# Nextomics/NextPolish2

Hardware: AMD Instinct MI355X
Metric: polished reference Mbp/s (whole node) at 30x HiFi + k21/k31; FASTA identical to oracle (higher is better)
Workload: dtype u8

## Files before the change

### nextpolish2_amd/csrc/np2_ctx.hpp

```cpp
#pragma once
#include "../../include/np2.h"
#include "np2_abi.hpp"
#include "np2_common.hpp"
#include "np2_kernels.hpp"
#include "np2_hostcpu.hpp"

#include <algorithm>
#include <chrono>
#include <cstdio>
#include <cstdlib>
#include <cstring>
#include <map>
#include <memory>
#include <exception>
#include <mutex>
#include <stdexcept>
#include <string>
#include <vector>

namespace np2h {

using namespace np2;


// ... 446 lines not shown
    DevBuf<uint16_t> keep_ks;
    DevBuf<uint32_t> long_list;
    DevBuf<uint64_t> bt_path;
    DevBuf<uint64_t> chunk_st;
    uint32_t chunk_epoch = 0;
    DevBuf<uint32_t> tile_cur, tile_n, tile_scan, tile_scanb, tile_nn, tile_nr, tile_noff, tile_roff;
    uint32_t tile_cap = TILE_CAP;
    uint32_t bucket_cap = 0;
    DevBuf<uint2> nrec;
    DevBuf<uint8_t> votebuf;
    DevBuf<uint32_t> band, band_n, band_off, row_cnt;
    DevBuf<int64_t> run_gain, tile_gain;
    DevBuf<uint8_t> out_snap;
    DevBuf<uint8_t> run_flag;
    uint32_t deep_min = 65536;
    DevBuf<uint32_t> lq_list, hbits;
    DevBuf<uint16_t> tile_pidx;
    bool pidx_valid = false;
    DevBuf<ReadInfo> rinfo;
    DevBuf<uint32_t> lqc, lqoff;
    DevBuf<uint8_t> pflag;
    DevBuf<uint32_t> dp_list;
    DevBuf<uint16_t> pf_slots;
    DevBuf<uint32_t> pf_bad, pf_bad2;
    DevBuf<uint64_t> pf_prof;
    bool front_fused = false;
    struct Hooks {
        bool front_unfused = false, pf_prof = false, edge_sort = false;
        bool test_misspeculate = false, shard_spec_log = false, phase_profile = false, exact_grow = false, no_speculate = false;
        bool has_grow_guess = false;
        uint32_t grow_guess = 0;
        bool has_pf_cap = false, has_pf_cap_big = false, has_pf_halo = false, has_pf_cov_max = false;
        uint32_t pf_cap = 0, pf_cap_big = 0, pf_halo = 0, pf_cov_max = 0;
        void read() {
            auto on = [](const char *n) { return getenv(n) != nullptr; };
            auto u32 = [](const char *n, bool &has, uint32_t &v) {
                if (const char *e = getenv(n)) has = true, v = (uint32_t)atol(e);
            };
            front_unfused = on("NP2_FRONT_UNFUSED"), pf_prof = on("NP2_PF_PROF"), edge_sort = on("NP2_EDGE_SORT");
            test_misspeculate = on("NP2_TEST_MISSPECULATE");
            shard_spec_log = on("NP2_SHARD_SPEC_LOG"), phase_profile = on("NP2_PHASE_PROFILE"), exact_grow = on("NP2_EXACT_GROW");
            no_speculate = on("NP2_NO_SPECULATE");
            u32("NP2_TEST_GROW_GUESS", has_grow_guess, grow_guess);
            u32("NP2_PF_CAP", has_pf_cap, pf_cap), u32("NP2_PF_CAP_BIG", has_pf_cap_big, pf_cap_big);
            u32("NP2_PF_HALO", has_pf_halo, pf_halo), u32("NP2_PF_COV_MAX", has_pf_cov_max, pf_cov_max);
        }
    } hooks;
    bool pf_big = getenv("NP2_PF_BIG") != nullptr;
    uint32_t front_redos = 0;
    DevBuf<uint16_t> kscore_saved;
    DevBuf<uint8_t> sstr;
    DevBuf<uint64_t> soff;
    DevBuf<uint16_t> sscore;
};


namespace np2h {


enum Scal { S_ERR = 0, S_NNODES, S_NRUNS, S_BEST, S_PATHBEGIN, S_NRAW, S_NREG, S_DUP, S_LAST0, S_LAST1, S_GAIN0,
            S_GAIN1, S_DEEP, S_NDPLIST, S_NRECH, S_NGROUPS, S_NLONG, S_NLQ, S_PF, S_M0, S_M1, S_M2, S_M3, S_NC, S_SB, S_GROW,
            S_NBAD, S_PFOUT, S_PFGAIN0, S_PFGAIN1, S_PFEND0, S_PFEND1, S_NBAD2, S_NOKEY, S_COUNT = 34 };
static_assert(S_M1 % 2 == 0 && S_LAST0 % 2 == 0 && S_GAIN0 % 2 == 0 && S_PFGAIN0 % 2 == 0 && S_PFEND0 % 2 == 0,
              "64-bit device counters live in these slot pairs");

static constexpr int NP2_MAX_YAK = 15;
static constexpr uint32_t SCAL_TOTAL = 96;
static_assert(S_COUNT + 2 * (NP2_MAX_YAK + 2) <= SCAL_TOTAL && S_COUNT < 64, "round counters behind the posted block; the mailbox holds 64 words");

inline double thread_cpu_ms() {
    timespec ts;
    clock_gettime(CLOCK_THREAD_CPUTIME_ID, &ts);
    return ts.tv_sec * 1e3 + ts.tv_nsec * 1e-6;
}
struct WallTimer {
    np2_ctx *cx;
    const char *name;
    double t0, c0 = 0;
    WallTimer(np2_ctx *c, const char *n);
    ~WallTimer();
};

struct EventTimer {
    np2_ctx *cx;
    hipEvent_t a = nullptr, b = nullptr;
    bool on;
    EventTimer(np2_ctx *c, const char *name, bool always = false)
        : cx(c), on((always || c->stage_timing) && !tl_recorder()) {
        if (!on) return;
        (void)hipEventCreate(&a);
        (void)hipEventCreate(&b);
        (void)hipEventRecord(a, cx->stream);
        cx->pending_events.push_back({name, {a, b}});
    }
    ~EventTimer() {
// ... 233 lines not shown
```

### nextpolish2_amd/csrc/np2_graph.hip

```cpp
#include "np2_common.hpp"
#include "np2_kernels.hpp"
#include "np2_blockscan.hpp"
#include "np2_lookback.hpp"

namespace np2 {

__device__ __forceinline__ uint32_t block_excl_scan_256(uint32_t v, uint32_t *sh, uint32_t &total) {
    return block_excl_scan<OpAdd, 4>(v, sh, total);
}

__device__ uint64_t make_node_key(const np2_read_t *__restrict__ reads, const uint8_t *__restrict__ nib, uint64_t rec,
                                  uint32_t r) {
    const uint32_t col = (uint32_t)rec, t3 = (uint32_t)(rec >> 32);
    const np2_read_t rd = reads[r];
    const uint8_t *base = nib + rd.nib_off;
    const uint32_t ts = rd.aln_t_s;
    auto mk = [&](int64_t c, uint32_t t) -> AlignBase {
        if (c == -2) return ab_head(ts - 1, 0);
        if (c == -1) return ab_head(ts - 1, 1);
        const uint8_t nb = nib_at(base, (uint32_t)c);
        AlignBase a;
        a.q = nb & 7;
        a.t_pos = t;
        a.delta = 0;
        if (c > 0 && (nb & 8)) {
            uint16_t dl = 1;
            int64_t x = c - 1;
            while (x > 0 && (nib_at(base, (uint32_t)x) & 8)) {
                dl = (uint16_t)(dl + 1);
                --x;
            }
            a.delta = dl;
        }
        return a;
    };
    auto is_ins = [&](int64_t c) -> bool { return c > 0 && (nib_at(base, (uint32_t)c) & 8); };
    const int64_t c3 = col;
    const AlignBase b3 = mk(c3, t3);
    const uint32_t t2 = is_ins(c3) ? t3 : t3 - 1;
    const AlignBase b2 = mk(c3 - 1, t2);
    const uint32_t t1 = is_ins(c3 - 1) ? t2 : t2 - 1;
    const AlignBase b1 = mk(c3 - 2, t1);
    return ((uint64_t)b3.t_pos << 32) | ((uint64_t)node_bases(b1, b2, b3) << 16) | b1.delta;
}

__device__ __forceinline__ void k_tile_layout(const uint32_t np2_bid, const uint32_t np2_nb, uint32_t *__restrict__ tile_cur, uint32_t n_tiles,
                                                      uint32_t bucket_cap, uint32_t *__restrict__ tile_n,
                                                      uint32_t *__restrict__ tile_scan, uint32_t *__restrict__ tile_scanb,
                                                      const uint32_t *__restrict__ ovf_cnt, uint32_t *__restrict__ out) {
    __shared__ uint32_t sh[16];
    const uint32_t ta = block_scan_array<OpAdd>(
        n_tiles, sh, [&](uint32_t i) { return tile_cur[i]; },
        [&](uint32_t i, uint32_t pre, uint32_t v) {
            tile_scan[i] = pre;
            tile_n[i] = v;
        });
    const uint32_t tb = block_scan_array<OpAdd>(
        n_tiles, sh, [&](uint32_t i) { return min(tile_n[i], bucket_cap); },
        [&](uint32_t i, uint32_t pre, uint32_t) { tile_scanb[i] = pre; });
    const uint32_t mx = block_scan_array<OpMaxU32>(
        n_tiles, sh, [&](uint32_t i) { return tile_n[i]; }, [&](uint32_t i, uint32_t, uint32_t) { tile_cur[i] = 0; });
    if (threadIdx.x == 0) {
        tile_scan[n_tiles] = ta;
        tile_scanb[n_tiles] = tb;
        out[0] = ta;
        out[1] = mx;
        out[2] = *ovf_cnt;
    }
}

static constexpr uint32_t TLB_ITEMS = 4;
__device__ __forceinline__ void k_tile_layout_lb(const uint32_t np2_bid, const uint32_t np2_nb, Lookback lb, uint32_t n_blocks, uint32_t *__restrict__ tile_cur,
                                                        uint32_t n_tiles, uint32_t bucket_cap, uint32_t *__restrict__ tile_n,
                                                        uint32_t *__restrict__ tile_scan, uint32_t *__restrict__ tile_scanb,
                                                        const uint32_t *__restrict__ ovf_cnt, uint32_t *__restrict__ out,
                                                        uint32_t *__restrict__ err) {
// ... 67 lines not shown
        s_klo[i] = (uint32_t)k;
        s_v[i] = r;
        s_q[i] = (uint16_t)q;
        atomicAdd(&s_cnt[q], 1u);
    }
    __syncthreads();
    {
        const uint32_t q0 = tid * 4;
        const uint32_t c0 = s_cnt[q0], c1 = s_cnt[q0 + 1], c2 = s_cnt[q0 + 2], c3 = s_cnt[q0 + 3];
        uint32_t tot;
        const uint32_t l0 = block_excl_scan_256(c0 + c1 + c2 + c3, sh, tot);
        s_off[q0] = (uint16_t)l0, s_off[q0 + 1] = (uint16_t)(l0 + c0), s_off[q0 + 2] = (uint16_t)(l0 + c0 + c1), s_off[q0 + 3] = (uint16_t)(l0 + c0 + c1 + c2);
        s_cnt[q0] = 0, s_cnt[q0 + 1] = 0, s_cnt[q0 + 2] = 0, s_cnt[q0 + 3] = 0;
    }
    __syncthreads();
    for (uint32_t i = tid; i < n; i += 256) {
        const uint32_t q = s_q[i];
        s_idx[s_off[q] + atomicAdd(&s_cnt[q], 1u)] = (uint16_t)i;
    }
    if (tid < TILE / 16) pidx[(size_t)np2_bid * (TILE / 16) + tid] = s_off[tid * 16];
    __syncthreads();
    for (uint32_t d = tid; d < n; d += 256) {
        const uint32_t i = s_idx[d], q = s_q[i], b = s_off[q], m = s_cnt[q];
        const uint32_t klo = s_klo[i], v = s_v[i];
        uint32_t rank = 0;
        for (uint32_t e = b; e < b + m; ++e) {
            const uint32_t j = s_idx[e];
            const uint32_t kj = s_klo[j], vj = s_v[j];
            rank += (kj < klo || (kj == klo && vj < v)) ? 1u : 0u;
        }
        keys[a + b + rank] = ((uint64_t)(start + q) << 32) | klo;
        vals[a + b + rank] = v;
    }
}

__device__ __forceinline__ void k_gather_buckets(const uint32_t np2_bid, const uint32_t np2_nb, const np2_read_t *__restrict__ reads,
                                                        const uint8_t *__restrict__ nib,
                                                        const uint32_t *__restrict__ tile_n,
                                                        const uint32_t *__restrict__ tile_scanb, uint32_t bucket_cap,
                                                        const uint64_t *__restrict__ bkeys,
                                                        const uint32_t *__restrict__ bvals, uint64_t *__restrict__ keys,
                                                        uint32_t *__restrict__ vals) {
    const uint32_t n = min(tile_n[np2_bid], bucket_cap);
    const uint64_t a = (uint64_t)np2_bid * bucket_cap;
    const uint32_t dst = tile_scanb[np2_bid];
    for (uint32_t i = threadIdx.x; i < n; i += 256) {
        const uint32_t r = bvals[a + i];
        keys[dst + i] = make_node_key(reads, nib, bkeys[a + i], r);
        vals[dst + i] = r;
    }
}
__device__ __forceinline__ void k_gather_spill(const uint32_t np2_bid, const uint32_t np2_nb, const np2_read_t *__restrict__ reads, const uint8_t *__restrict__ nib,
                               const uint64_t *__restrict__ okeys, const uint32_t *__restrict__ ovals, uint32_t n,
                               uint64_t *__restrict__ keys, uint32_t *__restrict__ vals) {
    const uint32_t i = np2_bid * blockDim.x + threadIdx.x;
    if (i >= n) return;
    const uint32_t r = ovals[i];
    keys[i] = make_node_key(reads, nib, okeys[i], r);
    vals[i] = r;
}

__device__ __forceinline__ bool group_head(const uint64_t *__restrict__ keys, const uint32_t *__restrict__ vals,
                                           const uint8_t *__restrict__ alive, uint64_t i, uint64_t a, uint64_t b,
                                           uint32_t &cnt, uint32_t &mn) {
    const uint64_t k = keys[i];
    if (i > a && keys[i - 1] == k) return false;
// ... 456 lines not shown
                if (q0 + j < npos) {
                    cov[start + q0 + j] = cv[j];
                    node_off[start + q0 + j] = nbase + off[j];
                    emit[start + q0 + j] = em[j];
                }
        }
    }
    if (np2_bid == n_tiles - 1 && tid == 255) node_off[L] = nbase + off[4];
    if (max(max(cv[0], cv[1]), max(cv[2], cv[3])) >= deep_min) atomicOr(deep_flag, 1u);
    if (tid == 0) tile_gain[np2_bid] = s_gain[0] + s_gain[1] + s_gain[2] + s_gain[3];
    if (fast) {
        for (uint32_t i = tid; i < nn; i += 256) {
            const uint32_t kk = s_nkey[i], c = s_ncnt[i];
            const uint32_t o = nbase + i;
            nd.bases[o] = (uint16_t)(kk >> 16);
            nd.delta[o] = (uint16_t)kk;
            nd.count[o] = c;
            nrec[o] = make_uint2((kk >> 16) | (kk << 16), c);
        }
    }
}

uint32_t tile_scan_blocks(uint32_t n_tiles) { return (n_tiles + 256 * TLB_ITEMS - 1) / (256 * TLB_ITEMS); }
void launch_tile_layout(hipStream_t s, uint32_t *tile_cur, uint32_t n_tiles, uint32_t bucket_cap, uint32_t *tile_n,
                        uint32_t *tile_scan, uint32_t *tile_scanb, const uint32_t *ovf_cnt, uint32_t *out,
                        const Lookback *lb, uint32_t *err) {
    if (lb)
        NP2_LAUNCH(k_tile_layout_lb, dim3(tile_scan_blocks(n_tiles)), 256, s, *lb, tile_scan_blocks(n_tiles), tile_cur, n_tiles, bucket_cap, tile_n, tile_scan, tile_scanb, ovf_cnt, out, err);
    else
        NP2_LAUNCH(k_tile_layout, dim3(1), 1024, s, tile_cur, n_tiles, bucket_cap, tile_n, tile_scan, tile_scanb, ovf_cnt, out);
}
void launch_tile_sort(hipStream_t s, uint16_t *pidx, const np2_read_t *reads, const uint8_t *nib, const uint32_t *tile_n,
                      uint32_t n_tiles, uint32_t bucket_cap, uint32_t max_tile, uint64_t *keys, uint32_t *vals,
                      uint32_t *err) {
    const uint32_t ALL = 0xFFFFFFFFu;
    if (max_tile <= 1024) {
        NP2_LAUNCH(k_tile_sort<1024>, dim3(n_tiles), 256, s, pidx, reads, nib, tile_n, bucket_cap, keys, vals, err, 0u, ALL);
    } else {
        NP2_LAUNCH(k_tile_sort<1024>, dim3(n_tiles), 256, s, pidx, reads, nib, tile_n, bucket_cap, keys, vals, err, 0u, 1024u);
        if (max_tile <= 2048 && TILE_CAP > 2048)
            NP2_LAUNCH(k_tile_sort<2048>, dim3(n_tiles), 256, s, pidx, reads, nib, tile_n, bucket_cap, keys, vals, err, 1024u, ALL);
        else
            NP2_LAUNCH(k_tile_sort<TILE_CAP>, dim3(n_tiles), 256, s, pidx, reads, nib, tile_n, bucket_cap, keys, vals, err, 1024u, ALL);
    }
}
void launch_gather_buckets(hipStream_t s, const np2_read_t *reads, const uint8_t *nib, const uint32_t *tile_n,
                           const uint32_t *tile_scanb, uint32_t n_tiles, uint32_t bucket_cap, const uint64_t *bkeys,
                           const uint32_t *bvals, uint64_t *keys, uint32_t *vals) {
    NP2_LAUNCH(k_gather_buckets, dim3(n_tiles), 256, s, reads, nib, tile_n, tile_scanb, bucket_cap, bkeys, bvals, keys, vals);
}
void launch_gather_spill(hipStream_t s, const np2_read_t *reads, const uint8_t *nib, const uint64_t *okeys,
                         const uint32_t *ovals, uint32_t n, uint64_t *keys, uint32_t *vals) {
    if (n) NP2_LAUNCH(k_gather_spill, dim3((n + 255) / 256), 256, s, reads, nib, okeys, ovals, n, keys, vals);
}
void launch_tile_count(hipStream_t s, const uint64_t *keys, const uint32_t *vals, const uint32_t *tile_n,
                       const uint32_t *tile_scan, uint32_t bucket_cap, uint32_t n_tiles, const uint8_t *alive,
                       uint32_t *tile_nn, uint32_t *tile_nr) {
    NP2_LAUNCH(k_tile_count, dim3(n_tiles), 256, s, keys, vals, TileLayout{tile_n, tile_scan, bucket_cap}, alive, tile_nn, tile_nr);
}
void launch_tile_offsets(hipStream_t s, const uint32_t *tile_nn, const uint32_t *tile_nr, uint32_t n_tiles,
                         uint32_t *tile_noff, uint32_t *tile_roff, uint32_t *n_nodes, uint32_t *n_runs, uint32_t *reset,
                         uint32_t n_reset, const Lookback *lb, uint32_t *err, const long long *tile_gain,
                         unsigned long long *gain_total) {
    if (lb)
        NP2_LAUNCH(k_tile_offsets_lb, dim3(tile_scan_blocks(n_tiles)), 256, s, *lb, tile_scan_blocks(n_tiles), tile_nn, tile_nr, n_tiles, tile_noff, tile_roff, n_nodes, n_runs, reset, n_reset, err, tile_gain, gain_total);
    else
        NP2_LAUNCH(k_tile_offsets, dim3(1), 1024, s, tile_nn, tile_nr, n_tiles, tile_noff, tile_roff, n_nodes, n_runs, reset, n_reset, tile_gain, gain_total);
}
void launch_tile_write(hipStream_t s, const uint64_t *keys, const uint32_t *vals, const uint32_t *tile_n,
                       const uint32_t *tile_scan, uint32_t bucket_cap, const uint32_t *tile_noff, const uint32_t *tile_roff,
                       uint32_t n_tiles, const uint8_t *alive, uint32_t L, NodeArrays nd, uint2 *nrec, uint32_t *node_off,
                       uint32_t *run_start, const np2_read_t *reads, const uint32_t *tile_rd_off, const uint32_t *tile_rd,
                       int32_t *cov, const uint8_t *refnib, uint32_t *emit, long long *tile_gain, uint32_t *deep_flag, uint32_t deep_min,
                       uint8_t *pflag) {
    NP2_LAUNCH(k_tile_write, dim3(n_tiles), 256, s, keys, vals, TileLayout{tile_n, tile_scan, bucket_cap}, tile_noff, tile_roff, alive, L, n_tiles, nd, nrec, node_off, run_start, reads, tile_rd_off, tile_rd, cov, refnib, emit, tile_gain, deep_flag, (int32_t)deep_min, pflag);
}
// ... 3 lines not shown
```

### nextpolish2_amd/csrc/np2_host.cpp

```cpp
#include "../../include/np2.h"
#include "np2_common.hpp"
#include "np2_kernels.hpp"
#include "np2_ctx.hpp"
#include "np2_phase_host.hpp"

#include <algorithm>
#include <atomic>
#include <thread>
#include <chrono>
#include <cstdio>
#include <cstdlib>
#include <cstring>
#include <map>
#include <mutex>
#include <stdexcept>
#include <string>
#include <unordered_map>
#include <unordered_set>
#include <future>
#include <functional>
#include <vector>

using namespace np2;

// ... 617 lines not shown
            launch_diff_reads(s, c->descs.p, NCH, c->nib.p, (const uint64_t *)c->refnib.p, c->refnib.p, c->refnib.p + c->ref_stride, c->ref_stride, L,
                              cx->keys_raw.p, cx->vals_raw.p, cx->tile_cur.p, n_tiles, bcap, buckets, (uint32_t)ovf_cap,
                              cx->scal.p + S_M3, c->ckpt.p, cx->chunk_st.p, cx->chunk_epoch, cx->scal.p + S_ERR);
        }
        {
            EventTimer t(cx, "sort_exceptions");
            const bool wide = n_tiles >= 2048;
            Lookback lb{};
            if (wide) lb = next_lookback(cx, tile_scan_blocks(n_tiles));
            launch_tile_layout(s, cx->tile_cur.p, n_tiles, bcap, cx->tile_n.p, cx->tile_scan.p, cx->tile_scanb.p,
                               cx->scal.p + S_M3, cx->scal.p + S_M0, wide ? &lb : nullptr, cx->scal.p + S_ERR);
        }
        std::vector<uint32_t> sc = fetch_scal(cx);
        static const bool test_fail = getenv("NP2_TEST_DENSE_LB_FAIL") != nullptr;
        if (test_fail && attempt == 0 && !precount) sc[S_ERR] |= LB_ERR;
        if ((sc[S_ERR] & LB_ERR) && !precount) {
            precount = true;
            continue;
        }
        if (sc[S_ERR] & ~2u) check_region_err(cx, sc[S_ERR] & ~2u);
        if (sc[S_ERR] & 2u)
            throw Np2Error(NP2_E_ARG, "packed read inconsistent with its descriptor (n_cols / aln_t_e / terminator)");
        if (sc[S_M2] > ovf_cap) {
            ovf_cap = (uint64_t)sc[S_M2] * 5 / 4 + 65536;
            continue;
        }
        T = sc[S_M0];
        if (T >= 0xFFFFFFF0u) throw Np2Error(NP2_E_NOMEM, "too many exception nodes");
        cx->tmp.ensure(prim_temp_bytes(std::max<size_t>({(size_t)T + 1, (size_t)L + 2, (size_t)R + 1})));
        EventTimer t(cx, "sort_exceptions");
        if (sc[S_M2] == 0) {
            cx->tile_pidx.ensure((size_t)n_tiles * (TILE / 16) + 64);
            launch_tile_sort(s, cx->tile_pidx.p, c->reads.p, c->nib.p, cx->tile_n.p, n_tiles, bcap, sc[S_M1], cx->keys_raw.p,
                             cx->vals_raw.p, cx->scal.p + S_ERR);
            cx->bucket_cap = bcap;
            cx->pidx_valid = true;
        } else {
            cx->keys.ensure((size_t)T + 1);
            cx->vals.ensure((size_t)T + 1);
            const uint32_t nb = T - sc[S_M2];
            launch_gather_buckets(s, c->reads.p, c->nib.p, cx->tile_n.p, cx->tile_scanb.p, n_tiles, bcap, cx->keys_raw.p,
                                  cx->vals_raw.p, cx->keys.p, cx->vals.p);
            launch_gather_spill(s, c->reads.p, c->nib.p, cx->keys_raw.p + buckets, cx->vals_raw.p + buckets, sc[S_M2],
                                cx->keys.p + nb, cx->vals.p + nb);
            unsigned pos_bits = 1;
            while ((1ull << pos_bits) < (uint64_t)L + 1) ++pos_bits;
            prim_op(cx, [=](hipStream_t st) {
                if (prim_sort_pairs_u64_u32(st, cx->tmp.p, cx->tmp.cap, cx->keys.p, cx->keys_raw.p, cx->vals.p, cx->vals_raw.p,
                                            T, 32 + pos_bits))
                    throw Np2Error(NP2_E_DEVICE, "rocprim radix_sort_pairs failed");
            });
            cx->bucket_cap = 0;
            cx->pidx_valid = false;
        }
        return;
    }
    throw Np2Error(NP2_E_NOMEM, "exception buffer kept overflowing");
}

void build_graph(np2_ctx *cx, np2_contig *c, uint32_t T, uint32_t &n_nodes, uint32_t &n_runs) {
    hipStream_t s = cx->stream;
    const uint32_t L = c->L;
    const uint32_t n_tiles = (L + TILE - 1) >> TILE_SHIFT;
    EventTimer t(cx, "build_graph");
    cx->npos.ensure(T + 1);
    cx->nbases.ensure(T + 1);
    cx->ndelta.ensure(T + 1);
// ... 192 lines not shown
        launch_pf_tile(s, a);
        if (prof) {
            auto st = d2h(cx, cx->pf_prof.p, (size_t)n_tiles * 8);
            double sum[8] = {0}, mx[8] = {0};
            size_t cnt = 0;
            for (uint32_t t = 0; t < n_tiles; ++t) {
                const uint64_t *q = st.data() + (size_t)t * 8;
                if (!q[7] || !q[0]) continue;
                ++cnt;
                for (int i = 1; i < 8; ++i) {
                    const double d = (double)(q[i] - q[i - 1]);
                    sum[i] += d, mx[i] = std::max(mx[i], d);
                }
            }
            {
                auto tn = d2h(cx, cx->tile_n.p, n_tiles);
                uint32_t h[6] = {0};
                for (uint32_t v : tn) ++h[v <= 480 ? 0 : v <= 960 ? 1 : v <= 1440 ? 2 : v <= 1920 ? 3 : v <= 3584 ? 4 : 5];
                fprintf(stderr, "[pf_prof] records per tile <=480 / 960 / 1440 / 1920 / 3584 / more: %u %u %u %u %u %u; ", h[0], h[1], h[2], h[3], h[4], h[5]);
            }
            fprintf(stderr, "listed for the middle / the big variant: %u / %u; ", d2h(cx, cx->scal.p + S_NBAD, 1)[0], d2h(cx, cx->scal.p + S_NBAD2, 1)[0]);
            fprintf(stderr, "tiles %zu of %u; mean / max clocks per phase (loads, cover+nodes, offsets+sort, DP, reduce, count+scan, write):", cnt, n_tiles);
            for (int i = 1; i < 8; ++i) fprintf(stderr, " %.0f/%.0f", cnt ? sum[i] / cnt : 0.0, mx[i]);
            fprintf(stderr, "\n");
        }
        const bool wide = n_tiles >= 2048;
        Lookback lb{};
        if (wide) lb = next_lookback(cx, tile_scan_blocks(n_tiles));
        launch_tile_offsets(s, cx->tile_nn.p, cx->tile_nr.p, n_tiles, cx->tile_noff.p, cx->tile_roff.p, M_p, n_lq,
                            cx->scal.p + S_BEST, S_NLQ + 1 - S_BEST, wide ? &lb : nullptr, cx->scal.p + S_ERR,
                            (const long long *)cx->tile_gain.p, (unsigned long long *)(cx->scal.p + S_PFGAIN0));
        launch_pf_compact(s, n_tiles, cx->pf_slots.p, cx->tile_scan.p, cx->tile_nn.p, cx->tile_noff.p, cx->tile_roff.p,
                          cx->cns_pos.p, cx->cns_base.p, cx->cns_cls.p, cx->lq_nothead.p, cx->lq_list.p, cb.lq_cap,
                          cx->scal.p + S_ERR, cx->scal.p + S_PF, cx->scal.p + S_PFOUT, cx->scal.p + S_NBAD, cx->scal.p + S_NBAD2);
    }
    lq_regions_issue(cx, cb, M_p, n_lq);
}

void pass_front_issue(np2_ctx *cx, np2_contig *c, uint32_t T, int pass, bool force_unfused = false) {
    cx->front_fused = !force_unfused && front_can_fuse(cx);
    if (!cx->front_fused || cx->trace) {
        uint32_t n_nodes = 0, n_runs = 0;
        {
            WallTimer w(cx, "wall_graph");
            build_graph(cx, c, T, n_nodes, n_runs);
        }
        trace_graph(cx, c, pass, n_nodes);
        if (!cx->front_fused) {
            consensus_and_regions_issue(cx, c, n_nodes, n_runs, T);
            return;
        }
    }
    pass_front_fused_issue(cx, c, T);
}
void consensus_and_regions_finish(np2_ctx *cx, np2_contig *c, uint32_t T, int pass, uint32_t &M, uint32_t &n_reg, bool whole_contig = true) {
    const uint32_t *M_p = cx->eoff.p + c->L;
    std::vector<uint32_t> sc = fetch_scal(cx, cx->scal.p + S_M0, M_p);
    if (cx->front_fused) {
        const int64_t total = (int64_t)(((uint64_t)sc[S_PFGAIN1] << 32) | sc[S_PFGAIN0]);
        const int64_t end_rel = (int64_t)(((uint64_t)sc[S_PFEND1] << 32) | sc[S_PFEND0]);
        const bool negative = end_rel <= SCORE_NEG / 2 || total + end_rel < 0;
        if (sc[S_PFOUT] & PF_NEED_BIG) cx->pf_big = true;
        if ((sc[S_PFOUT] & PF_REDO) || negative) {
            ++cx->front_redos;
            cx->timing.host.push_back({"front_redo", 1.0f});
            pass_front_issue(cx, c, T, pass, true);
            sc = fetch_scal(cx, cx->scal.p + S_M0, M_p);
        }
    }
    check_region_err(cx, sc[S_ERR]);
    if (!cx->front_fused && sc[S_BEST] == 0xFFFFFFFFu && !whole_contig)
        throw Np2Error(NP2_E_UNSUPPORTED,
                       "best path score is negative at the end of a shard (the reference's default node is chosen by the whole "
                       "contig's score): polish this contig unsharded");
    M = sc[S_M0];
    if (M == 0) throw Np2Error(NP2_E_REFPANIC, "reference would panic: empty consensus");
    n_reg = sc[S_NRAW] ? sc[S_NREG] : 0;
}

void extract_candidates(np2_ctx *cx, np2_contig *c, uint32_t n_reg, uint16_t min_kmer_count, int pass,
                        PassCounts &pc) {
    hipStream_t s = cx->stream;
    const uint32_t R = c->R;
    REFPANIC_IF(cx->yaks.empty(), "index out of bounds: opt.yak[0]");
    if ((uint64_t)n_reg * LQSEQ_MAX_CAN_COUNT >= 0xFFFFFFF0ull) throw Np2Error(NP2_E_NOMEM, "too many LQ regions");
    const uint32_t NC_cap = n_reg * LQSEQ_MAX_CAN_COUNT;
    static const uint64_t exact_from = getenv("NP2_CAND_EXACT_FROM") ? strtoull(getenv("NP2_CAND_EXACT_FROM"), nullptr, 10) : (1ull << 28);
    const bool exact_bytes = c->n_cols >= exact_from && !cx->trace;
    uint32_t SB_cap = (uint32_t)std::min<uint64_t>(c->n_cols + 64, 0xFFFFFFF0ull);
    cx->mval.ensure(R + 2);
    cx->smin.ensure(R + 2);
    cx->pj.ensure(R + 2);
    cx->pcount.ensure(R + 2);
    cx->rinfo.ensure(R + 2);
    cx->reg_ncand.ensure(n_reg + 2);
// ... 1372 lines not shown
```

### nextpolish2_amd/csrc/np2_kernels.hpp

```cpp
#pragma once
#include <cstddef>
#include <cstdint>
#include <hip/hip_runtime.h>
#include "../../include/np2.h"
#include "np2_lookback.hpp"
#include "np2_launch.hpp"

namespace np2 {

static constexpr uint32_t TILE_SHIFT = 10;
static constexpr uint32_t TILE = 1u << TILE_SHIFT;
static constexpr uint32_t TILE_CAP = 4096;

static constexpr uint32_t DENSE_COLS = 4096;
struct ChunkDesc {
    uint64_t nib_off;
    uint64_t ckbase;
    uint32_t read, ts;
    uint32_t c0, ncols;
    uint32_t first_chunk;
    uint32_t aln_t_e, nck;
    uint32_t pad0;
    uint32_t pad[4];
};
// ... 148 lines not shown
                          uint16_t min_count, uint16_t *out, bool own_strings);
void launch_cand_score(hipStream_t s, const YakDev &y, const uint32_t *cand_seq_off, const uint8_t *cand_seq,
                       const uint64_t *cand_kmer, const uint32_t *n_cand_p, uint32_t cand_cap, uint16_t min_count,
                       uint16_t *kscore, uint32_t *long_list, uint32_t *n_long);


void launch_pair_count(hipStream_t s, const np2_read_t *reads, uint32_t R, const uint8_t *alive,
                       const uint32_t *lq_start, const uint32_t *lq_end, uint32_t n_reg, const int32_t *smin,
                       uint32_t *pj, uint32_t *pcount, const uint64_t *ck_off, ReadInfo *rinfo);
void launch_scan_lb_excl(hipStream_t s, const Lookback &lb, const uint32_t *in, uint32_t *out, uint32_t n, bool write_end,
                          uint32_t *err);
uint32_t scan_lb_blocks(uint64_t n);
void launch_scan_small_excl(hipStream_t s, const uint32_t *in, uint32_t *out, uint32_t n, const uint32_t *n_dev,
                            uint32_t *total_out, bool write_end);
void launch_scan_small_incl(hipStream_t s, const int32_t *in, int32_t *out, uint32_t n, const uint32_t *n_dev);
void launch_scan_small_min(hipStream_t s, const int32_t *in, int32_t *out, uint32_t n, const uint32_t *n_dev);
void launch_region_measure(hipStream_t s, const CandPtrs &c, uint32_t n_reg, uint32_t *kept_read, uint32_t *kept_len,
                           uint32_t *kept_col, uint32_t *reg_ncand, uint32_t *reg_bytes, uint32_t *reg_maxlen,
                           uint32_t *blk_sum);
uint32_t cand_offsets_blocks(uint32_t n_reg);
void launch_cand_offsets(hipStream_t s, const uint32_t *blk_sum, uint32_t n_reg, uint32_t *blk_coff, uint32_t *blk_soff,
                         uint32_t *cand_off, uint32_t *reg_soff, uint32_t *n_cand, uint32_t *n_bytes, uint32_t *grow,
                         const Lookback *lb = nullptr, uint32_t *err = nullptr);
void launch_region_write(hipStream_t s, const CandPtrs &c, uint32_t n_reg, const uint32_t *kept_read,
                         const uint32_t *kept_len, const uint32_t *kept_col, const uint32_t *reg_ncand,
                         const uint32_t *reg_bytes, const uint32_t *blk_coff, const uint32_t *blk_soff, uint32_t *cand_off,
                         uint32_t *reg_soff, uint32_t cand_cap, uint32_t seq_cap, uint32_t *cand_order, uint64_t *cand_kmer,
                         uint32_t *cand_seq_off, uint8_t *cand_seq);

uint32_t tile_scan_blocks(uint32_t n_tiles);
void launch_tile_layout(hipStream_t s, uint32_t *tile_cur, uint32_t n_tiles, uint32_t bucket_cap, uint32_t *tile_n,
                        uint32_t *tile_scan, uint32_t *tile_scanb, const uint32_t *ovf_cnt, uint32_t *out,
                        const Lookback *lb = nullptr, uint32_t *err = nullptr);
void launch_tile_sort(hipStream_t s, uint16_t *pidx, const np2_read_t *reads, const uint8_t *nib, const uint32_t *tile_n,
                      uint32_t n_tiles, uint32_t bucket_cap, uint32_t max_tile, uint64_t *keys, uint32_t *vals,
                      uint32_t *err);
void launch_gather_buckets(hipStream_t s, const np2_read_t *reads, const uint8_t *nib, const uint32_t *tile_n,
                           const uint32_t *tile_scanb, uint32_t n_tiles, uint32_t bucket_cap, const uint64_t *bkeys,
                           const uint32_t *bvals, uint64_t *keys, uint32_t *vals);
void launch_gather_spill(hipStream_t s, const np2_read_t *reads, const uint8_t *nib, const uint64_t *okeys,
                         const uint32_t *ovals, uint32_t n, uint64_t *keys, uint32_t *vals);
void launch_tile_count(hipStream_t s, const uint64_t *keys, const uint32_t *vals, const uint32_t *tile_n,
                       const uint32_t *tile_scan, uint32_t bucket_cap, uint32_t n_tiles, const uint8_t *alive,
                       uint32_t *tile_nn, uint32_t *tile_nr);
void launch_tile_offsets(hipStream_t s, const uint32_t *tile_nn, const uint32_t *tile_nr, uint32_t n_tiles,
                         uint32_t *tile_noff, uint32_t *tile_roff, uint32_t *n_nodes, uint32_t *n_runs, uint32_t *reset,
                         uint32_t n_reset, const Lookback *lb = nullptr, uint32_t *err = nullptr,
                         const long long *tile_gain = nullptr, unsigned long long *gain_total = nullptr);
void launch_tile_write(hipStream_t s, const uint64_t *keys, const uint32_t *vals, const uint32_t *tile_n,
                       const uint32_t *tile_scan, uint32_t bucket_cap, const uint32_t *tile_noff, const uint32_t *tile_roff,
                       uint32_t n_tiles, const uint8_t *alive, uint32_t L, NodeArrays nd, uint2 *nrec, uint32_t *node_off,
                       uint32_t *run_start, const np2_read_t *reads, const uint32_t *tile_rd_off, const uint32_t *tile_rd,
                       int32_t *cov, const uint8_t *refnib, uint32_t *emit, long long *tile_gain, uint32_t *deep_flag, uint32_t deep_min,
                       uint8_t *pflag);

static constexpr uint32_t PF_CAP = 960;
static constexpr uint32_t PF_HALO = 64;
static constexpr uint32_t PF_CAP_MID = 2048;
static constexpr uint32_t PF_CAP_BIG = 3584;
static constexpr uint32_t PF_COV_MAX = 8192;
static constexpr uint32_t PF_REDO = 1u;
static constexpr uint32_t PF_NEED_BIG = 2u;
struct PfTile {
    const uint64_t *keys;
    const uint32_t *vals;
    const uint32_t *tile_n, *tile_scan;
    const uint16_t *pidx;
    const uint8_t *alive;
    const np2_read_t *reads;
    const uint32_t *tile_rd_off, *tile_rd;
    const uint8_t *refnib;
    uint16_t *slots;
    uint32_t *tile_cnt, *tile_lq;
    long long *tile_gain;
    uint32_t *flags, *n_bad, *bad_list, *n_bad2, *bad_list2;
    long long *end_rel;
    unsigned long long *gain_total;
    unsigned long long *prof;
    uint32_t L, n_tiles, bucket_cap;
    uint32_t cap_lim, cap_lim_big, halo_lim, cov_max;
    uint32_t big_enabled;
};
uint64_t pf_slot_entries(uint32_t n_tiles, uint64_t T);
void launch_pf_tile(hipStream_t s, const PfTile &a);
void launch_pf_compact(hipStream_t s, uint32_t n_tiles, const uint16_t *slots, const uint32_t *tile_scan, const uint32_t *tile_cnt,
                       const uint32_t *tile_coff, const uint32_t *tile_lqoff, uint32_t *cns_pos, uint8_t *cns_base,
                       uint8_t *cns_cls, uint8_t *lq_nothead, uint32_t *lq_list, uint32_t lq_cap, uint32_t *err, uint32_t *flags,
                       uint32_t *flags_out, uint32_t *n_bad, uint32_t *n_bad2);

struct RegionTables {
    const uint32_t *cand_off;
    const uint32_t *order;
    uint16_t *kscore;
    const uint32_t *seq_off;
    const uint8_t *seq;
    uint32_t n_reg;
};
struct RechPtrs {
    const void *groups;
    const uint32_t *job_off;
    const uint32_t *rech;
    const uint32_t *cand_off;
    const uint32_t *keep_list;
    const uint32_t *seq_off;
    const uint8_t *seq;
    const uint8_t *cns_base;
    uint32_t n_groups;
};
void launch_vote_phase(hipStream_t s, const RegionTables &rt, bool asref, bool use_all, const uint32_t *lq_start,
                       uint32_t own_lo, uint32_t own_hi, uint8_t *reg_lable, uint8_t *grp, uint32_t *ecount, int32_t *ref_w,
                       uint8_t *ref_seen, uint8_t *bad, uint32_t *first_reg, uint32_t *err);
void launch_vote_counts(hipStream_t s, const uint32_t *first_reg, const uint8_t *bad, uint32_t R, uint32_t *out);
void launch_edges_write(hipStream_t s, const RegionTables &rt, const uint8_t *reg_lable, const uint8_t *grp,
                        const uint32_t *ecount, const uint32_t *eoff, uint64_t *ekey, uint32_t *eval);
static constexpr uint32_t EDGE_BAND = 256;
void launch_edges_row(hipStream_t s, const RegionTables &rt, const uint8_t *grp, const uint32_t *ecount, const uint32_t *pj,
                      const uint32_t *pcount, const uint8_t *alive, uint32_t R, uint32_t *band, uint32_t *row_n, uint32_t *ovf);
void launch_band_emit(hipStream_t s, const uint32_t *band, uint32_t R, const uint32_t *row_off, uint64_t *ukey, uint32_t *uw,
                      uint32_t *n_out, uint64_t key_add = 0);
void launch_vote_rows_count(hipStream_t s, const uint32_t *band, const uint32_t *row_n, const uint8_t *bad, bool use_all, uint32_t R,
                            uint32_t *cnt, uint32_t *nokey);
// ... 66 lines not shown
```

### nextpolish2_amd/csrc/np2_passfront.hip

```cpp
#include "np2_common.hpp"
#include "np2_kernels.hpp"
#include "np2_blockscan.hpp"

namespace np2 {

static constexpr uint32_t PF_COUNT_BITS = 14;
static constexpr uint32_t PF_IDX_MASK = (1u << PF_COUNT_BITS) - 1;
static constexpr uint32_t PF_VISITED = 0x80000000u;
static constexpr uint32_t PF_N0_VISITED = 0x8000u;
static constexpr uint32_t PF_N0_WEAK = 0x4000u;
static constexpr uint32_t PF_N0_STRONG = 0x2000u;
static constexpr int32_t PF_NEG = -(1 << 30);

__device__ __forceinline__ uint8_t pf_ref_code(const uint8_t *__restrict__ refnib, uint32_t p) {
    return (refnib[p >> 1] >> (4 * (p & 1))) & 7;
}
template <int I> __device__ __forceinline__ uint32_t pf_quad_bcast(uint32_t v) {
    return (uint32_t)__builtin_amdgcn_mov_dpp((int)v, I | (I << 2) | (I << 4) | (I << 6), 0xF, 0xF, true);
}
__device__ __forceinline__ void pf_n0_key(uint32_t p, uint32_t c2, uint32_t c1, uint32_t c0, uint32_t &b, uint32_t &d) {
    if (p >= 2) {
        b = (c2 << 8) | (c1 << 4) | c0, d = 0;
    } else if (p == 1) {
        b = 0x0F00u | (c1 << 4) | c0, d = 1;
// ... 707 lines not shown
        A.tile_lq[t] = s_flag[3];
        A.tile_gain[t] = s_gain[0] + s_gain[1] + s_gain[2] + s_gain[3];
        const bool last_clean = t + 1 == A.n_tiles && s_off[L - 1 - start + 1] == s_off[L - 1 - start];
        if (s_flag[4] || last_clean) *A.end_rel = s_endrel;
        if (t == 0) *A.gain_total = 0;
    }
}

__device__ __forceinline__ void k_pf_tile(const uint32_t np2_bid, const uint32_t np2_nb, PfTile A) {
    pf_tile_body<PF_CAP, PF_HALO, 0>(xcd_order(np2_bid, np2_nb), A);
}
__device__ __forceinline__ void k_pf_tile_mid(const uint32_t np2_bid, const uint32_t np2_nb, PfTile A) {
    const uint32_t nb = *A.n_bad;
    for (uint32_t i = np2_bid; i < nb; i += np2_nb) {
        pf_tile_body<PF_CAP_MID, PF_HALO, 1>(A.bad_list[i], A);
        __syncthreads();
    }
}
__device__ __forceinline__ void k_pf_tile_big(const uint32_t np2_bid, const uint32_t np2_nb, PfTile A) {
    const uint32_t nb = *A.n_bad2;
    for (uint32_t i = np2_bid; i < nb; i += np2_nb) {
        pf_tile_body<PF_CAP_BIG, TILE, 2>(A.bad_list2[i], A);
        __syncthreads();
    }
}

__device__ __forceinline__ void k_pf_compact(const uint32_t np2_bid, const uint32_t np2_nb, const uint16_t *__restrict__ slots,
                                             const uint32_t *__restrict__ tile_scan, const uint32_t *__restrict__ tile_cnt,
                                             const uint32_t *__restrict__ tile_coff, const uint32_t *__restrict__ tile_lqoff,
                                             uint32_t *__restrict__ cns_pos, uint8_t *__restrict__ cns_base,
                                             uint8_t *__restrict__ cns_cls, uint8_t *__restrict__ lq_nothead,
                                             uint32_t *__restrict__ lq_list, uint32_t lq_cap, uint32_t *__restrict__ err,
                                             uint32_t *__restrict__ flags, uint32_t *__restrict__ flags_out,
                                             uint32_t *__restrict__ n_bad, uint32_t *__restrict__ n_bad2) {
    __shared__ uint32_t s_w[4];
    const uint32_t t = np2_bid, tid = threadIdx.x, lane = tid & 63, wv = tid >> 6;
    if (t == 0 && tid == 0) {
        *flags_out = *flags;
        *flags = 0;
        *n_bad = 0;
        *n_bad2 = 0;
    }
    const uint32_t n = tile_cnt[t], o0 = tile_coff[t], start = t << TILE_SHIFT;
    const uint16_t *__restrict__ src = slots + pf_slot_off(tile_scan, t);
    uint32_t lqo = tile_lqoff[t];
    for (uint32_t i0 = 0; i0 < n; i0 += 256) {
        const uint32_t i = i0 + tid;
        uint32_t e = 0;
        bool lq = false;
        if (i < n) {
            e = src[i];
            const uint32_t cls = e >> 14;
            cns_pos[o0 + i] = start + (e & 0x7FFu);
            cns_base[o0 + i] = code_to_ascii((uint8_t)((e >> 11) & 7));
            cns_cls[o0 + i] = (uint8_t)cls;
            lq_nothead[o0 + i] = 0;
            lq = cls == CLS_LQ;
        }
        const uint64_t bal = __ballot(lq);
        if (lane == 0) s_w[wv] = (uint32_t)__builtin_popcountll(bal);
        __syncthreads();
        uint32_t before = 0, all = 0;
#pragma unroll
        for (uint32_t w = 0; w < 4; ++w) {
            const uint32_t x = s_w[w];
            all += x;
            if (w < wv) before += x;
        }
        if (lq) {
            const uint32_t k = lqo + before + __builtin_amdgcn_mbcnt_hi((uint32_t)(bal >> 32), __builtin_amdgcn_mbcnt_lo((uint32_t)bal, 0u));
            if (k < lq_cap)
                lq_list[k] = o0 + i;
            else
                atomicOr(err, LQ_LIST_ERR);
        }
        lqo += all;
        __syncthreads();
    }
}

uint64_t pf_slot_entries(uint32_t n_tiles, uint64_t T) { return (uint64_t)n_tiles * (TILE + 1) + 3 * T + 64; }
void launch_pf_tile(hipStream_t s, const PfTile &a) {
    NP2_LAUNCH(k_pf_tile, dim3(a.n_tiles), 256, s, a);
    NP2_LAUNCH(k_pf_tile_mid, dim3(std::min<uint32_t>(a.n_tiles, 256u)), 256, s, a);
    if (a.big_enabled) NP2_LAUNCH(k_pf_tile_big, dim3(std::min<uint32_t>(a.n_tiles, 64u)), 256, s, a);
}
void launch_pf_compact(hipStream_t s, uint32_t n_tiles, const uint16_t *slots, const uint32_t *tile_scan, const uint32_t *tile_cnt,
                       const uint32_t *tile_coff, const uint32_t *tile_lqoff, uint32_t *cns_pos, uint8_t *cns_base,
                       uint8_t *cns_cls, uint8_t *lq_nothead, uint32_t *lq_list, uint32_t lq_cap, uint32_t *err, uint32_t *flags,
                       uint32_t *flags_out, uint32_t *n_bad, uint32_t *n_bad2) {
    NP2_LAUNCH(k_pf_compact, dim3(n_tiles), 256, s, slots, tile_scan, tile_cnt, tile_coff, tile_lqoff, cns_pos, cns_base, cns_cls,
               lq_nothead, lq_list, lq_cap, err, flags, flags_out, n_bad, n_bad2);
}

}
```

Baseline: 4302.

## Keep tile-sort records in registers and rank through windowed shared memory

Adds a tile sort kernel that holds each thread's records (key low, value, bucket, slot) in registers instead of shared arrays. It batches the read metadata loads four at a time. Ranking within each bucket then runs over shared-memory windows of configurable size, so tiles up to 2048 records are handled in one launch instead of falling back to larger shared-memory variants. Register pressure rises with RPT=8, and records per thread are now capped with an error flag. It also adds profiling counters for the pass-front mid and big lists, which cost one extra write in the compact kernel.

Measured after the change: 4200. -2.4%, worse.

```diff
diff --git a/nextpolish2_amd/csrc/np2_ctx.hpp b/nextpolish2_amd/csrc/np2_ctx.hpp
--- a/nextpolish2_amd/csrc/np2_ctx.hpp
+++ b/nextpolish2_amd/csrc/np2_ctx.hpp
@@ -502,6 +502,8 @@
         uint32_t grow_guess = 0;
         bool has_pf_cap = false, has_pf_cap_big = false, has_pf_halo = false, has_pf_cov_max = false;
         uint32_t pf_cap = 0, pf_cap_big = 0, pf_halo = 0, pf_cov_max = 0;
+        bool has_sort_win = false;
+        uint32_t sort_win = 0;
         void read() {
             auto on = [](const char *n) { return getenv(n) != nullptr; };
             auto u32 = [](const char *n, bool &has, uint32_t &v) {
@@ -514,6 +516,7 @@
             u32("NP2_TEST_GROW_GUESS", has_grow_guess, grow_guess);
             u32("NP2_PF_CAP", has_pf_cap, pf_cap), u32("NP2_PF_CAP_BIG", has_pf_cap_big, pf_cap_big);
             u32("NP2_PF_HALO", has_pf_halo, pf_halo), u32("NP2_PF_COV_MAX", has_pf_cov_max, pf_cov_max);
+            u32("NP2_SORT_WIN", has_sort_win, sort_win);
         }
     } hooks;
     bool pf_big = getenv("NP2_PF_BIG") != nullptr;
@@ -530,7 +533,7 @@
 
 enum Scal { S_ERR = 0, S_NNODES, S_NRUNS, S_BEST, S_PATHBEGIN, S_NRAW, S_NREG, S_DUP, S_LAST0, S_LAST1, S_GAIN0,
             S_GAIN1, S_DEEP, S_NDPLIST, S_NRECH, S_NGROUPS, S_NLONG, S_NLQ, S_PF, S_M0, S_M1, S_M2, S_M3, S_NC, S_SB, S_GROW,
-            S_NBAD, S_PFOUT, S_PFGAIN0, S_PFGAIN1, S_PFEND0, S_PFEND1, S_NBAD2, S_NOKEY, S_COUNT = 34 };
+            S_NBAD, S_PFOUT, S_PFGAIN0, S_PFGAIN1, S_PFEND0, S_PFEND1, S_NBAD2, S_NOKEY, S_PFLMID, S_PFLBIG, S_COUNT = 36 };
 static_assert(S_M1 % 2 == 0 && S_LAST0 % 2 == 0 && S_GAIN0 % 2 == 0 && S_PFGAIN0 % 2 == 0 && S_PFEND0 % 2 == 0,
               "64-bit device counters live in these slot pairs");
 
diff --git a/nextpolish2_amd/csrc/np2_graph.hip b/nextpolish2_amd/csrc/np2_graph.hip
--- a/nextpolish2_amd/csrc/np2_graph.hip
+++ b/nextpolish2_amd/csrc/np2_graph.hip
@@ -9,12 +9,8 @@
     return block_excl_scan<OpAdd, 4>(v, sh, total);
 }
 
-__device__ uint64_t make_node_key(const np2_read_t *__restrict__ reads, const uint8_t *__restrict__ nib, uint64_t rec,
-                                  uint32_t r) {
+__device__ uint64_t make_node_key_at(const uint8_t *__restrict__ base, uint32_t ts, uint64_t rec) {
     const uint32_t col = (uint32_t)rec, t3 = (uint32_t)(rec >> 32);
-    const np2_read_t rd = reads[r];
-    const uint8_t *base = nib + rd.nib_off;
-    const uint32_t ts = rd.aln_t_s;
     auto mk = [&](int64_t c, uint32_t t) -> AlignBase {
         if (c == -2) return ab_head(ts - 1, 0);
         if (c == -1) return ab_head(ts - 1, 1);
@@ -42,6 +38,11 @@
     const uint32_t t1 = is_ins(c3 - 1) ? t2 : t2 - 1;
     const AlignBase b1 = mk(c3 - 2, t1);
     return ((uint64_t)b3.t_pos << 32) | ((uint64_t)node_bases(b1, b2, b3) << 16) | b1.delta;
+}
+__device__ uint64_t make_node_key(const np2_read_t *__restrict__ reads, const uint8_t *__restrict__ nib, uint64_t rec,
+                                  uint32_t r) {
+    const np2_read_t rd = reads[r];
+    return make_node_key_at(nib + rd.nib_off, rd.aln_t_s, rec);
 }
 
 __device__ __forceinline__ void k_tile_layout(const uint32_t np2_bid, const uint32_t np2_nb, uint32_t *__restrict__ tile_cur, uint32_t n_tiles,
@@ -175,6 +176,109 @@
         keys[a + b + rank] = ((uint64_t)(start + q) << 32) | klo;
         vals[a + b + rank] = v;
     }
+}
+
+template <uint32_t RPT>
+__device__ __forceinline__ void k_tile_sort_reg(const uint32_t np2_bid, const uint32_t np2_nb, uint16_t *__restrict__ pidx, const np2_read_t *__restrict__ reads,
+                                                       const uint8_t *__restrict__ nib, const uint32_t *__restrict__ tile_n,
+                                                       uint32_t bucket_cap, uint64_t *__restrict__ keys,
+                                                       uint32_t *__restrict__ vals, uint32_t *__restrict__ err,
+                                                       uint32_t n_above, uint32_t n_upto, uint32_t win) {
+    static_assert(256 * RPT <= 65536 && TILE <= 65536, "slot and position of a record share a word");
+    __shared__ uint32_t s_klo[TILE_SORT_WIN];
+    __shared__ uint32_t s_v[TILE_SORT_WIN];
+    __shared__ uint32_t s_cnt[TILE];
+    __shared__ uint16_t s_off[TILE];
+    __shared__ uint32_t sh[8];
+    const uint32_t n = tile_n[np2_bid], tid = threadIdx.x;
+    const uint64_t a = (uint64_t)np2_bid * bucket_cap;
+    if (n <= n_above || n > n_upto) return;
+    if (n > 256 * RPT) {
+        if (tid == 0) atomicOr(err, 8u);
+        return;
+    }
+    win = min(max(win, 1u), TILE_SORT_WIN);
+    const uint32_t start = np2_bid << TILE_SHIFT;
+    for (uint32_t i = tid; i < TILE; i += 256) s_cnt[i] = 0;
+    __syncthreads();
+    uint32_t rklo[RPT], rv[RPT], rqg[RPT], rank[RPT];
+    static_assert(RPT % 4 == 0, "records are fetched four at a time");
+#pragma unroll
+    for (uint32_t j = 0; j < RPT; ++j) rklo[j] = 0, rv[j] = 0, rqg[j] = 0, rank[j] = 0;
+#pragma unroll
+    for (uint32_t h = 0; h < RPT; h += 4) {
+        if (256 * h >= n) break;
+        uint64_t rrec[4], roff[4];
+        uint32_t rts[4];
+#pragma unroll
+        for (uint32_t j = 0; j < 4; ++j) {
+            const uint32_t i = tid + 256 * (h + j);
+            rv[h + j] = i < n ? vals[a + i] : 0u;
+            rrec[j] = i < n ? keys[a + i] : 0ull;
+        }
+#pragma unroll
+        for (uint32_t j = 0; j < 4; ++j) {
+            roff[j] = reads[rv[h + j]].nib_off;
+            rts[j] = reads[rv[h + j]].aln_t_s;
+        }
+#pragma unroll
+        for (uint32_t j = 0; j < 4; ++j) {
+            if (tid + 256 * (h + j) >= n) continue;
+            const uint64_t k = make_node_key_at(nib + roff[j], rts[j], rrec[j]);
+            uint32_t q = (uint32_t)(k >> 32) - start;
+            if (q >= TILE) {
+                atomicOr(err, 8u);
+                q = TILE - 1;
+            }
+            rklo[h + j] = (uint32_t)k, rqg[h + j] = q;
+            atomicAdd(&s_cnt[q], 1u);
+        }
+    }
+    __syncthreads();
+    {
+        const uint32_t q0 = tid * 4;
+        const uint32_t c0 = s_cnt[q0], c1 = s_cnt[q0 + 1], c2 = s_cnt[q0 + 2], c3 = s_cnt[q0 + 3];
+        uint32_t tot;
+        const uint32_t l0 = block_excl_scan_256(c0 + c1 + c2 + c3, sh, tot);
+        s_off[q0] = (uint16_t)l0, s_off[q0 + 1] = (uint16_t)(l0 + c0), s_off[q0 + 2] = (uint16_t)(l0 + c0 + c1), s_off[q0 + 3] = (uint16_t)(l0 + c0 + c1 + c2);
+        s_cnt[q0] = 0, s_cnt[q0 + 1] = 0, s_cnt[q0 + 2] = 0, s_cnt[q0 + 3] = 0;
+    }
+    __syncthreads();
+#pragma unroll
+    for (uint32_t j = 0; j < RPT; ++j)
+        if (tid + 256 * j < n) {
+            const uint32_t q = rqg[j];
+            rqg[j] = q | ((s_off[q] + atomicAdd(&s_cnt[q], 1u)) << 16);
+        }
+    if (tid < TILE / 16) pidx[(size_t)np2_bid * (TILE / 16) + tid] = s_off[tid * 16];
+    for (uint32_t w = 0; w < n; w += win) {
+        if (w) __syncthreads();
+#pragma unroll
+        for (uint32_t j = 0; j < RPT; ++j) {
+            const uint32_t g = (rqg[j] >> 16) - w;
+            if (tid + 256 * j < n && g < win) s_klo[g] = rklo[j], s_v[g] = rv[j];
+        }
+        __syncthreads();
+#pragma unroll
+        for (uint32_t j = 0; j < RPT; ++j)
+            if (tid + 256 * j < n) {
+                const uint32_t q = rqg[j] & 0xFFFFu, b = s_off[q];
+                const uint32_t lo = max(b, w), hi = min(b + s_cnt[q], w + win);
+                const uint32_t klo = rklo[j], v = rv[j];
+                for (uint32_t e = lo; e < hi; ++e) {
+                    const uint32_t kj = s_klo[e - w], vj = s_v[e - w];
+                    rank[j] += (kj < klo || (kj == klo && vj < v)) ? 1u : 0u;
+                }
+            }
+    }
+#pragma unroll
+    for (uint32_t j = 0; j < RPT; ++j)
+        if (tid + 256 * j < n) {
+            const uint32_t q = rqg[j] & 0xFFFFu;
+            const uint64_t d = a + s_off[q] + rank[j];
+            keys[d] = ((uint64_t)(start + q) << 32) | rklo[j];
+            vals[d] = rv[j];
+        }
 }
 
 __device__ __forceinline__ void k_gather_buckets(const uint32_t np2_bid, const uint32_t np2_nb, const np2_read_t *__restrict__ reads,
@@ -697,16 +801,15 @@
 }
 void launch_tile_sort(hipStream_t s, uint16_t *pidx, const np2_read_t *reads, const uint8_t *nib, const uint32_t *tile_n,
                       uint32_t n_tiles, uint32_t bucket_cap, uint32_t max_tile, uint64_t *keys, uint32_t *vals,
-                      uint32_t *err) {
+                      uint32_t *err, uint32_t win) {
     const uint32_t ALL = 0xFFFFFFFFu;
     if (max_tile <= 1024) {
-        NP2_LAUNCH(k_tile_sort<1024>, dim3(n_tiles), 256, s, pidx, reads, nib, tile_n, bucket_cap, keys, vals, err, 0u, ALL);
+        NP2_LAUNCH(k_tile_sort_reg<4>, dim3(n_tiles), 256, s, pidx, reads, nib, tile_n, bucket_cap, keys, vals, err, 0u, ALL, win);
+    } else if (max_tile <= 2048) {
+        NP2_LAUNCH(k_tile_sort_reg<8>, dim3(n_tiles), 256, s, pidx, reads, nib, tile_n, bucket_cap, keys, vals, err, 0u, ALL, win);
     } else {
-        NP2_LAUNCH(k_tile_sort<1024>, dim3(n_tiles), 256, s, pidx, reads, nib, tile_n, bucket_cap, keys, vals, err, 0u, 1024u);
-        if (max_tile <= 2048 && TILE_CAP > 2048)
-            NP2_LAUNCH(k_tile_sort<2048>, dim3(n_tiles), 256, s, pidx, reads, nib, tile_n, bucket_cap, keys, vals, err, 1024u, ALL);
-        else
-            NP2_LAUNCH(k_tile_sort<TILE_CAP>, dim3(n_tiles), 256, s, pidx, reads, nib, tile_n, bucket_cap, keys, vals, err, 1024u, ALL);
+        NP2_LAUNCH(k_tile_sort_reg<8>, dim3(n_tiles), 256, s, pidx, reads, nib, tile_n, bucket_cap, keys, vals, err, 0u, 2048u, win);
+        NP2_LAUNCH(k_tile_sort<TILE_CAP>, dim3(n_tiles), 256, s, pidx, reads, nib, tile_n, bucket_cap, keys, vals, err, 2048u, ALL);
     }
 }
 void launch_gather_buckets(hipStream_t s, const np2_read_t *reads, const uint8_t *nib, const uint32_t *tile_n,
diff --git a/nextpolish2_amd/csrc/np2_host.cpp b/nextpolish2_amd/csrc/np2_host.cpp
--- a/nextpolish2_amd/csrc/np2_host.cpp
+++ b/nextpolish2_amd/csrc/np2_host.cpp
@@ -673,7 +673,8 @@
         if (sc[S_M2] == 0) {
             cx->tile_pidx.ensure((size_t)n_tiles * (TILE / 16) + 64);
             launch_tile_sort(s, cx->tile_pidx.p, c->reads.p, c->nib.p, cx->tile_n.p, n_tiles, bcap, sc[S_M1], cx->keys_raw.p,
-                             cx->vals_raw.p, cx->scal.p + S_ERR);
+                             cx->vals_raw.p, cx->scal.p + S_ERR,
+                             cx->hooks.has_sort_win ? std::min(std::max(cx->hooks.sort_win, 1u), TILE_SORT_WIN) : TILE_SORT_WIN);
             cx->bucket_cap = bcap;
             cx->pidx_valid = true;
         } else {
@@ -932,7 +933,8 @@
                             (const long long *)cx->tile_gain.p, (unsigned long long *)(cx->scal.p + S_PFGAIN0));
         launch_pf_compact(s, n_tiles, cx->pf_slots.p, cx->tile_scan.p, cx->tile_nn.p, cx->tile_noff.p, cx->tile_roff.p,
                           cx->cns_pos.p, cx->cns_base.p, cx->cns_cls.p, cx->lq_nothead.p, cx->lq_list.p, cb.lq_cap,
-                          cx->scal.p + S_ERR, cx->scal.p + S_PF, cx->scal.p + S_PFOUT, cx->scal.p + S_NBAD, cx->scal.p + S_NBAD2);
+                          cx->scal.p + S_ERR, cx->scal.p + S_PF, cx->scal.p + S_PFOUT, cx->scal.p + S_NBAD, cx->scal.p + S_NBAD2,
+                          cx->scal.p + S_PFLMID);
     }
     lq_regions_issue(cx, cb, M_p, n_lq);
 }
@@ -961,6 +963,8 @@
         const int64_t end_rel = (int64_t)(((uint64_t)sc[S_PFEND1] << 32) | sc[S_PFEND0]);
         const bool negative = end_rel <= SCORE_NEG / 2 || total + end_rel < 0;
         if (sc[S_PFOUT] & PF_NEED_BIG) cx->pf_big = true;
+        cx->timing.host.push_back({"pf_listed_mid", (float)sc[S_PFLMID]});
+        cx->timing.host.push_back({"pf_listed_big", (float)sc[S_PFLBIG]});
         if ((sc[S_PFOUT] & PF_REDO) || negative) {
             ++cx->front_redos;
             cx->timing.host.push_back({"front_redo", 1.0f});
diff --git a/nextpolish2_amd/csrc/np2_kernels.hpp b/nextpolish2_amd/csrc/np2_kernels.hpp
--- a/nextpolish2_amd/csrc/np2_kernels.hpp
+++ b/nextpolish2_amd/csrc/np2_kernels.hpp
@@ -204,9 +204,10 @@
 void launch_tile_layout(hipStream_t s, uint32_t *tile_cur, uint32_t n_tiles, uint32_t bucket_cap, uint32_t *tile_n,
                         uint32_t *tile_scan, uint32_t *tile_scanb, const uint32_t *ovf_cnt, uint32_t *out,
                         const Lookback *lb = nullptr, uint32_t *err = nullptr);
+static constexpr uint32_t TILE_SORT_WIN = 1024;
 void launch_tile_sort(hipStream_t s, uint16_t *pidx, const np2_read_t *reads, const uint8_t *nib, const uint32_t *tile_n,
                       uint32_t n_tiles, uint32_t bucket_cap, uint32_t max_tile, uint64_t *keys, uint32_t *vals,
-                      uint32_t *err);
+                      uint32_t *err, uint32_t win = TILE_SORT_WIN);
 void launch_gather_buckets(hipStream_t s, const np2_read_t *reads, const uint8_t *nib, const uint32_t *tile_n,
                            const uint32_t *tile_scanb, uint32_t n_tiles, uint32_t bucket_cap, const uint64_t *bkeys,
                            const uint32_t *bvals, uint64_t *keys, uint32_t *vals);
@@ -258,7 +259,7 @@
 void launch_pf_compact(hipStream_t s, uint32_t n_tiles, const uint16_t *slots, const uint32_t *tile_scan, const uint32_t *tile_cnt,
                        const uint32_t *tile_coff, const uint32_t *tile_lqoff, uint32_t *cns_pos, uint8_t *cns_base,
                        uint8_t *cns_cls, uint8_t *lq_nothead, uint32_t *lq_list, uint32_t lq_cap, uint32_t *err, uint32_t *flags,
-                       uint32_t *flags_out, uint32_t *n_bad, uint32_t *n_bad2);
+                       uint32_t *flags_out, uint32_t *n_bad, uint32_t *n_bad2, uint32_t *listed_out);
 
 struct RegionTables {
     const uint32_t *cand_off;
diff --git a/nextpolish2_amd/csrc/np2_passfront.hip b/nextpolish2_amd/csrc/np2_passfront.hip
--- a/nextpolish2_amd/csrc/np2_passfront.hip
+++ b/nextpolish2_amd/csrc/np2_passfront.hip
@@ -763,11 +763,13 @@
                                              uint8_t *__restrict__ cns_cls, uint8_t *__restrict__ lq_nothead,
                                              uint32_t *__restrict__ lq_list, uint32_t lq_cap, uint32_t *__restrict__ err,
                                              uint32_t *__restrict__ flags, uint32_t *__restrict__ flags_out,
-                                             uint32_t *__restrict__ n_bad, uint32_t *__restrict__ n_bad2) {
+                                             uint32_t *__restrict__ n_bad, uint32_t *__restrict__ n_bad2,
+                                             uint32_t *__restrict__ listed_out) {
     __shared__ uint32_t s_w[4];
     const uint32_t t = np2_bid, tid = threadIdx.x, lane = tid & 63, wv = tid >> 6;
     if (t == 0 && tid == 0) {
         *flags_out = *flags;
+        listed_out[0] = *n_bad, listed_out[1] = *n_bad2;
         *flags = 0;
         *n_bad = 0;
         *n_bad2 = 0;
@@ -819,9 +821,9 @@
 void launch_pf_compact(hipStream_t s, uint32_t n_tiles, const uint16_t *slots, const uint32_t *tile_scan, const uint32_t *tile_cnt,
                        const uint32_t *tile_coff, const uint32_t *tile_lqoff, uint32_t *cns_pos, uint8_t *cns_base,
                        uint8_t *cns_cls, uint8_t *lq_nothead, uint32_t *lq_list, uint32_t lq_cap, uint32_t *err, uint32_t *flags,
-                       uint32_t *flags_out, uint32_t *n_bad, uint32_t *n_bad2) {
+                       uint32_t *flags_out, uint32_t *n_bad, uint32_t *n_bad2, uint32_t *listed_out) {
     NP2_LAUNCH(k_pf_compact, dim3(n_tiles), 256, s, slots, tile_scan, tile_cnt, tile_coff, tile_lqoff, cns_pos, cns_base, cns_cls,
-               lq_nothead, lq_list, lq_cap, err, flags, flags_out, n_bad, n_bad2);
+               lq_nothead, lq_list, lq_cap, err, flags, flags_out, n_bad, n_bad2, listed_out);
 }
 
 }
```
